# nh13/DWGSIM

Hardware: AMD Instinct MI355X
Metric: M read-pairs/sec (2x150 bp PE) (higher is better)
Workload: dtype u8

## Files before the change

dwgsim_amd/csrc/dw_host.cpp:

```cpp
#include <hip/hip_runtime.h>
#include <math.h>
#include <stdio.h>
#include <stdlib.h>
#include <string.h>
#include <limits.h>
#include <ctype.h>
#include <stdarg.h>
#include <stdint.h>
#include <sys/mman.h>
#include <mutex>
#include <thread>
#include <string>
#include <vector>
#include <algorithm>
#include <array>
#include <stddef.h>
#include <type_traits>
#include "../../include/dwgsim_hip.h"
#include "dw_kernels.hpp"
#include "dw_launch.hpp"
#include "dw_mutin.hpp"
#include "dw_mem.hpp"

using namespace dw;
// ... 1916 lines not shown
    if (c->depth_on && !c->truth_on) { size_t ends = 0; for (int j = 0; j < 2; ++j) if (p.length[j] > 0) ends += n_pairs; P.t_ends = sizeof(TruthEnd) * ends; }
    if (c->truth_on) {
        P.t_qname_max = fixed_max + 120;
        size_t ends = 0, bytes = 0;
        for (int j = 0; j < 2; ++j) if (p.length[j] > 0) { ends += n_pairs; bytes += (size_t)n_pairs * (size_t)(P.t_qname_max + fixed_max + 3 + 10 + 2 + 1 + 10 + 11 + 6 + 11 + 1 + 15 * (size_t)p.length[j]); }
        if (c->truth_md) for (int j = 0; j < 2; ++j) if (p.length[j] > 0) bytes += (size_t)n_pairs * (size_t)(12 + 10 + 2 * (size_t)p.length[j] + 1);
        if (run.truth_bytes) bytes = (size_t)run.truth_bytes;
        else if (c->dbg.truth_cap >= 0 && c->truth_md) bytes = (size_t)std::max<int64_t>(c->dbg.truth_cap, 64);
        P.cap[3] = bytes;
        const bool bfast_src = !L.a.p.has_bwa;
        for (int q = 0; q < (bfast_src ? 1 : f.lpp); ++q) {
            const size_t src_cap = P.cap[bfast_src ? 2 : q];
            P.t_nl[q] = sizeof(uint32_t) * ((src_cap + 4095) / 4096 + 1); P.t_rec[q] = sizeof(uint32_t) * ((bfast_src ? ends : (size_t)n_pairs) + 2);
        }
        P.t_ends = sizeof(TruthEnd) * ends; P.t_len = sizeof(uint32_t) * (ends + 1); P.t_blk = sizeof(uint32_t) * (nblk + 1);
        for (int t = 0; t < N_STREAMS; ++t) if ((uint64_t)P.cap[t] >> 32) P.too_many = true;
    }
    P.block_rand = sizeof(uint32_t) * nblk;
    if (!f.split) P.status = 4 * sizeof(uint64_t) * nblk;
    else { P.split_state = sizeof(uint32_t) * (size_t)f.lds_words * SIM_THREADS * nblk; P.split_hand = 16 * (size_t)SIM_THREADS * nblk; P.split_agg = 16 * nblk; P.split_pre = 32 * nblk; P.split_chunk = 32 * (nblk / 1024 + 1); }
    P.meta = sizeof(uint32_t) * ((size_t)n_pairs + 8);
    P.fail_summ = ((size_t)((n_pairs + 256ull * 64 - 1) / (256ull * 64)) * 4 + 2) * sizeof(uint64_t);
    P.scratch = f.dt == 2 || (f.dt < 2 && f.nthr == SIM_THREADS_LONG);
    if (P.scratch) {
        const int cu_per_xcd = (c->n_cu >= 64 && c->n_cu % 8 == 0) ? c->n_cu / 8 : c->n_cu;
        const bool ion = p.data_type == 2;
        const int per_cu = sim_blocks_per_cu(f.lds, ion ? 8 : 32);
        P.flow_slots = c->dbg.flow_slots > 0 ? c->dbg.flow_slots : cu_per_xcd * per_cu;
        if ((uint64_t)P.flow_slots > (uint64_t)nblk) P.flow_slots = (int32_t)nblk;
        if (ion) {
            const size_t slot_bytes = (size_t)flow_words_per_lane(f.lds_words) * (size_t)SIM_THREADS * sizeof(uint32_t);
            const size_t fit = std::max<size_t>(1, ((size_t)4 << 30) / (slot_bytes * 8));
            if ((size_t)P.flow_slots > fit) P.flow_slots = (int32_t)fit;
        }
        const size_t words = (ion ? (size_t)flow_words_per_lane(f.lds_words) * (size_t)SIM_THREADS : (size_t)f.lds_words * (size_t)SIM_THREADS_LONG) * (size_t)P.flow_slots * 8;
        P.flow_scratch = words * sizeof(uint32_t); P.flow_free = sizeof(uint64_t) * (256 + 8 * nblk);
    }
    P.segs = sizeof(SimSeg) * L.segs.size();
    if (c->gzip_on) {
        size_t chunks = 0;
        for (int t = 0; t < N_STREAMS; ++t) { P.gz_chunks[t] = (size_t)gz_chunks(P.cap[t]); chunks += P.gz_chunks[t]; if (P.cap[t]) P.gz_cap[t] = (size_t)gz_capacity(P.cap[t]); }
        P.gz_status = sizeof(uint64_t) * (chunks ? chunks : 1);
    }
    return P;
}

static int sim_reserve(dwgsim_hip_ctx_t *c, int slot, const SimPlan &P)
{
    Slot &sl = c->slot[slot]; DevMem *out = c->out[slot];
    if (sl.fetch_in_flight) { HIPC(c, hipStreamWaitEvent(c->stream.get(), sl.ev_fetched.get(), 0)); bool grows = false; for (int t = 0; t < N_STREAMS; ++t) if (P.cap[t] + 64 > out[t].cap() && (t < 3 || P.cap[t])) grows = true; if (grows) HIPC(c, hipEventSynchronize(sl.ev_fetched.get())); sl.fetch_in_flight = false; }
    for (int t = 0; t < 3; ++t) if (ensure(c, out[t], P.cap[t] + 64)) return DWGSIM_HIP_ERR_DEVICE;
    if (P.cap[3] && (ensure(c, out[3], P.cap[3] + 64) || ensure(c, c->t_nl[0], P.t_nl[0]) || ensure(c, c->t_nl[1], P.t_nl[1]) || ensure(c, c->t_rec[0], P.t_rec[0]) || ensure(c, c->t_rec[1], P.t_rec[1]) ||
                     ensure(c, c->t_len, P.t_len) || ensure(c, c->t_blk, P.t_blk))) return DWGSIM_HIP_ERR_DEVICE;
    if (ensure(c, c->t_ends, P.t_ends)) return DWGSIM_HIP_ERR_DEVICE;
    if (ensure(c, c->block_rand, P.block_rand) || ensure(c, c->status_all, P.status) ||
        ensure(c, c->split_state, P.split_state) || ensure(c, c->split_hand, P.split_hand) || ensure(c, c->split_agg, P.split_agg) || ensure(c, c->split_pre, P.split_pre) || ensure(c, c->split_chunk, P.split_chunk) ||
        ensure(c, c->meta, P.meta) || ensure(c, c->fail_summ, P.fail_summ) || ensure(c, c->flow_scratch, P.flow_scratch) || ensure(c, c->flow_free, P.flow_free) || ensure(c, sl.segs, P.segs)) return DWGSIM_HIP_ERR_DEVICE;
    HIPC(c, sl.h_segs.reserve(P.segs, P.segs + 64 * sizeof(SimSeg)));
    for (int t = 0; t < N_STREAMS; ++t) if (P.gz_cap[t] && ensure(c, sl.gz_out[t], P.gz_cap[t] + 64)) return DWGSIM_HIP_ERR_DEVICE;
    return ensure(c, sl.gz_status, P.gz_status);
}

static ChainSet sim_chain(dwgsim_hip_ctx_t *c, Slot &sl, const dwgsim_hip_range_t *r, int n, const SimRun &run)
{
    if (run.again) return ChainSet{sl.d_rerun_chain.get<uint64_t>(), 1, 1, 0};
    const dwgsim_hip_range_t *r_first = nullptr, *r_last = nullptr;
    for (int q = 0; q < n; ++q) if (r[q].n_pairs) { if (!r_first) r_first = &r[q]; r_last = &r[q]; }
    if (!r_first) { r_first = &r[0]; r_last = &r[n - 1]; }
    const bool continues = c->chain_contig == r_first->contig && c->chain_next_ii == r_first->first_ii && r_first->first_ii != 0;
    const ChainSet ch{c->d_chain.get<uint64_t>(), run.rand_base != DWGSIM_HIP_RAND_CHAIN ? 1 : 0, (c->has_carry_override || !continues) ? 1 : 0, c->has_carry_override ? c->carry_override : 0};
    c->has_carry_override = false; c->chain_contig = r_last->contig; c->chain_next_ii = r_last->first_ii + r_last->n_pairs;
    if (sl.ranges.data() != r) sl.ranges.assign(r, r + n);
    return ch;
}

static int sim_launch(dwgsim_hip_ctx_t *c, int slot, Launch &L, const SimPlan &P, const ChainSet &ch, const SimRun &run)
{
    Slot &sl = c->slot[slot]; SimArgs &a = L.a; const SimForm &f = L.f; uint64_t *cnt = sl.counters.dev();
    const uint64_t n_pairs = L.n_pairs, rand_base = run.rand_base; const uint32_t nblk = L.nblk;
    for (int t = 0; t < N_STREAMS; ++t) sl.out_bytes[t] = sl.gz_bytes[t] = 0;
    sl.n_pairs = n_pairs; sl.empty = n_pairs == 0; sl.truth_timed = false;
    if (n_pairs == 0) { if (ch.set_rand || ch.set_carry) launch_chain_set(c->stream.get(), ch.words, rand_base, ch.set_rand, ch.carry, ch.set_carry); return DWGSIM_HIP_OK; }
    uint32_t opens = 0; for (const SimSeg &s : L.segs) opens |= s.contig_start;
    memcpy(sl.h_segs.get(), L.segs.data(), P.segs);
    HIPC(c, hipMemcpyAsync(sl.segs.get(), sl.h_segs.get(), P.segs, hipMemcpyHostToDevice, c->stream.get()));
    a.segs = sl.segs.get<SimSeg>(); a.n_seg = (int32_t)L.segs.size(); a.n_blocks = nblk; a.n_pairs = n_pairs; a.chain = ch.words; a.lb_shift = P.lb_shift;
    a.meta = c->meta.get<uint32_t>(); a.block_rand = c->block_rand.get<uint32_t>(); a.counters = cnt;
    for (int t = 0; t < 3; ++t) a.out[t] = c->out[slot][t].get<uint8_t>();
    for (int j = 0; j < 4; ++j) a.status[j] = f.split ? nullptr : c->status_all.get<uint64_t>() + (size_t)j * (size_t)nblk;
    if (f.split) { a.split_state = c->split_state.get<uint32_t>(); a.split_hand = c->split_hand.get<uint32_t>(); a.split_agg = c->split_agg.get<uint32_t>(); a.split_pre = c->split_pre.get<uint64_t>(); a.split_chunk = c->split_chunk.get<uint64_t>(); }
    if (P.scratch) { a.flow_scratch = c->flow_scratch.get<uint32_t>(); a.flow_free = c->flow_free.get<uint64_t>(); a.flow_slots = P.flow_slots; }
    sl.group = c->handles[(size_t)L.g->first_handle].group;
    launch_init(c->stream.get(), cnt, (uint32_t)N_COUNTERS, a.status[0], f.split ? 0 : 4 * (uint64_t)nblk, a.flow_free, a.flow_free ? 256 + 8 * (uint64_t)nblk : 0,
                ch.words, rand_base, ch.set_rand, ch.carry, ch.set_carry);
    HIPC(c, hipEventRecord(sl.ev_k0.get(), c->stream.get()));
    c->dbg.sim_form = (int64_t)f.nthr << 20 | f.lpp << 16 | f.out << 12 | f.dt << 8 | f.wr << 4 | f.split;
    if (!launch_simulate(c->stream.get(), a, f)) { c->err = "simulate: no k_simulate instance for this form"; return DWGSIM_HIP_ERR_FAILED; }
    HIPC(c, hipEventRecord(sl.ev_k1.get(), c->stream.get()));
    sl.cap_mult = c->flow_cap_mult;
    if (!run.again) launch_failrule(c->stream.get(), a.meta, n_pairs, opens, c->fail_summ.get<uint64_t>(), cnt, c->d_chain.get<uint64_t>());
    const bool depth = c->depth_on && !run.again && L.g->depth_valid && !L.g->depth_pos.empty();
    if (P.cap[3] || depth) {
        TruthArgs t; memset(&t, 0, sizeof t);
        sl.truth_timed = true;
        HIPC(c, hipEventRecord(sl.ev_t0.get(), c->stream.get()));
        t.lpp = f.lpp; t.bfast = a.p.has_bwa ? 0 : 1; t.prefix_len = c->read_prefix.empty() ? 0 : (int32_t)c->read_prefix.size() + 1; t.qname_max = P.t_qname_max;
        DepthArgs dp; dp.pos = L.g->mem.d_depth_pos.get<int32_t>(); dp.n = (uint32_t)L.g->depth_pos.size(); dp.cnt = L.g->mem.d_depth_cnt.get<unsigned long long>();
        for (int q = 0; P.cap[3] && q < (t.bfast ? 1 : f.lpp); ++q) {
            const int st = t.bfast ? 2 : q;
            t.src[q] = a.out[st]; t.src_bytes[q] = &cnt[text_len_counter(st)]; t.src_cap[q] = P.cap[st];
            t.nl_count[q] = c->t_nl[q].get<uint32_t>(); t.rec[q] = c->t_rec[q].get<uint32_t>(); t.n_rec[q] = t.bfast ? n_pairs * (uint64_t)f.lpp : n_pairs;
        }
        t.ends = c->t_ends.get<TruthEnd>(); t.line_len = c->t_len.get<uint32_t>(); t.blk = c->t_blk.get<uint32_t>();
        t.out = c->out[slot][3].get<uint8_t>(); t.cap = P.cap[3]; t.total = &cnt[text_len_counter(3)];
        t.md = c->truth_md ? 1 : 0; t.ref = L.g->mem.d_ref.get(); t.fit = &cnt[TRUTH_FIT_COUNTER];
        if (P.cap[3]) launch_truth(c->stream.get(), a, t, depth ? &dp : nullptr);
        else launch_truth_depth(c->stream.get(), a, t, dp);
        HIPC(c, hipEventRecord(sl.ev_t1.get(), c->stream.get()));
    }
    if (c->gzip_on) {
        HIPC(c, hipMemsetAsync(sl.gz_status.get(), 0, P.gz_status, c->stream.get()));
        size_t off = 0;
        for (int t = 0; t < N_STREAMS; ++t) {
            if (P.cap[t] == 0) continue;
            launch_gzip(c->stream.get(), c->out[slot][t].get<uint8_t>(), &cnt[gz_src_len_counter(t, c->truth_md)], P.cap[t], sl.gz_out[t].get<uint8_t>(), P.gz_cap[t], sl.gz_status.get<uint64_t>() + off,
                        &cnt[gz_ticket_counter(t)], &cnt[gz_len_counter(t)], &cnt[STATUS_COUNTER], c->d_crc_table.get<uint32_t>(), c->d_crc_shift.get<uint32_t>());
            off += P.gz_chunks[t];
        }
    }
    HIPC(c, hipEventRecord(sl.ev_end.get(), c->stream.get()));
    HIPC(c, hipGetLastError());
    HIPC(c, hipMemcpyAsync(sl.counters.host(), cnt, N_COUNTERS * sizeof(uint64_t), hipMemcpyDeviceToHost, c->stream.get()));
    HIPC(c, hipEventRecord(sl.ev_done.get(), c->stream.get()));
    sl.pending = true;
    return DWGSIM_HIP_OK;
}

static int sim_enqueue(dwgsim_hip_ctx_t *c, const dwgsim_hip_range_t *r, int n, int slot, const SimRun &run)
{
    if (!c || slot < 0 || slot >= DWGSIM_HIP_SLOTS) { if (c) c->err = "bad simulate arguments"; return DWGSIM_HIP_ERR_ARG; }
    if (c->slot[slot].pending) { c->err = "simulate: the slot still holds a batch that was not waited for"; return DWGSIM_HIP_ERR_STATE; }
    Launch L;
    if (const int rc = sim_resolve(c, r, n, L)) return rc;
    HIPC(c, hipSetDevice(c->device));
    const SimPlan P = sim_plan(c, L, run);
    if (P.too_many) { c->err = "too many pairs in one call"; return DWGSIM_HIP_ERR_ARG; }
    if (L.n_pairs) { if (const int rc = sim_reserve(c, slot, P)) return rc; }
    if (L.n_pairs && c->depth_on && !run.again) { if (const int rc = depth_prepare(c, *L.g)) return rc; }
    return sim_launch(c, slot, L, P, sim_chain(c, c->slot[slot], r, n, run), run);
}

int dwgsim_hip_simulate_ranges_async(dwgsim_hip_ctx_t *c, const dwgsim_hip_range_t *r, int n, uint64_t rand_base, int slot) { return sim_enqueue(c, r, n, slot, SimRun{rand_base, false, 0}); }

int dwgsim_hip_simulate_async(dwgsim_hip_ctx_t *c, int contig, uint64_t first_ii, uint64_t n_pairs, uint64_t rand_base, int slot)
{
    dwgsim_hip_range_t r; memset(&r, 0, sizeof r); r.contig = contig; r.first_ii = first_ii; r.n_pairs = n_pairs;
    return dwgsim_hip_simulate_ranges_async(c, &r, 1, rand_base, slot);
}

static int sim_rerun(dwgsim_hip_ctx_t *c, int slot, uint64_t truth_bytes)
{
    static const int kept[7] = {fail_seg_counter(0), fail_seg_counter(1), fail_seg_counter(2), fail_seg_counter(3), ABORT_COUNTER, CARRY_COUNTER, CHAIN_BASE_COUNTER};
    Slot &sl = c->slot[slot]; uint64_t *h = sl.counters.host();
    uint64_t keep[7]; for (int q = 0; q < 7; ++q) keep[q] = h[kept[q]];
    if (const int rc = sim_enqueue(c, sl.ranges.data(), (int)sl.ranges.size(), slot, SimRun{h[CHAIN_BASE_COUNTER], true, truth_bytes})) return rc;
    HIPC(c, hipEventSynchronize(sl.ev_done.get())); sl.pending = false;
    for (int q = 0; q < 7; ++q) h[kept[q]] = keep[q];
    return DWGSIM_HIP_OK;
}

static int batch_verdict(dwgsim_hip_ctx_t *c, const uint64_t *h)
{
    const uint64_t st = h[STATUS_COUNTER];
    if (st & REGIONS_BIT) { c->err = "dwgsim-hip: no fragment placement satisfied the target regions (-x) after 2^20 tries (the reference would not terminate)\n"; return DWGSIM_HIP_ERR_FAILED; }
    if (st & FLOW_ROOM_BIT) { c->err = "dwgsim-hip: a read outgrew its buffer (or degenerated) in the flow-error model\n"; return DWGSIM_HIP_ERR_FAILED; }
    if ((st & ~(GZIP_ROOM_BIT | TRUTH_ERR_BIT | TRUTH_ROOM_BIT)) || h[ABORT_COUNTER]) return fail_attempts(c);
    if (st & GZIP_ROOM_BIT) { c->err = "dwgsim-hip: the gzip output buffer is too small for this text\n"; return DWGSIM_HIP_ERR_FAILED; }
    if (st & TRUTH_ERR_BIT) { c->err = "dwgsim-hip: the truth SAM could not be made (a read's record or alignment could not be replayed)\n"; return DWGSIM_HIP_ERR_FAILED; }
    if (st & TRUTH_ROOM_BIT) { c->err = "dwgsim-hip: the truth SAM did not fit its buffer\n"; return DWGSIM_HIP_ERR_FAILED; }
    return DWGSIM_HIP_OK;
}

int dwgsim_hip_wait(dwgsim_hip_ctx_t *c, int slot, dwgsim_hip_batch_t *out)
{
    if (!c || slot < 0 || slot >= DWGSIM_HIP_SLOTS) { if (c) c->err = "bad slot"; return DWGSIM_HIP_ERR_ARG; }
    Slot &sl = c->slot[slot];
    if (out) memset(out, 0, sizeof *out);
    if (sl.empty) { sl.pending = false; return DWGSIM_HIP_OK; }
    if (!sl.pending) { c->err = "wait: no batch was enqueued on this slot"; return DWGSIM_HIP_ERR_STATE; }
    HIPC(c, hipSetDevice(c->device));
    HIPC(c, hipEventSynchronize(sl.ev_done.get()));
    sl.pending = false;
    const uint64_t *h = sl.counters.host();
    if ((h[STATUS_COUNTER] & FLOW_ROOM_BIT) && !(h[STATUS_COUNTER] & ~(FLOW_ROOM_BIT | GZIP_ROOM_BIT)) && c->prm.data_type == 2) {
        while (h[STATUS_COUNTER] & FLOW_ROOM_BIT) {
            if (sl.cap_mult >= c->flow_cap_mult) {
                if ((int64_t)flow_base_capacity(c) * (int64_t)c->flow_cap_mult * 2 > (int64_t)FLOW_CAP_MAX) break;
                c->flow_cap_mult *= 2;
            }
            if (const int rc = sim_rerun(c, slot, 0)) return rc;
        }
    }
    if (h[STATUS_COUNTER] == TRUTH_ROOM_BIT && !h[ABORT_COUNTER]) {
        const uint64_t need = h[text_len_counter(3)];
        if (need + 64 >= (1ull << 32)) { c->err = "dwgsim-hip: the truth SAM of one batch would pass 4 GiB with its MD strings (deletions are spelled out): use smaller batches\n"; return DWGSIM_HIP_ERR_UNSUP; }
        if (const int rc = sim_rerun(c, slot, need)) return rc;
        ++c->dbg.truth_reruns;
        if (h[STATUS_COUNTER] & TRUTH_ROOM_BIT) { c->err = "dwgsim-hip: the truth SAM did not fit the room its own scan asked for\n"; return DWGSIM_HIP_ERR_FAILED; }
    }
    if (const int rc = batch_verdict(c, h)) return rc;
    for (int t = 0; t < N_STREAMS; ++t) { sl.out_bytes[t] = h[text_len_counter(t)]; sl.gz_bytes[t] = h[gz_len_counter(t)]; }
    if (!c->truth_on) sl.out_bytes[3] = sl.gz_bytes[3] = 0;
    if (c->dbg.phases) {
        uint64_t tot = 0; for (int k = 0; k < N_PHASES; ++k) tot += h[phase_counter(k)];
        fprintf(stderr, "[phases]");
// ... 332 lines not shown
```

dwgsim_amd/csrc/dw_kernels.hpp:

```cpp
#pragma once
#include <stdint.h>

namespace dw {

constexpr int PAIRS_PER_BLOCK = 128;
constexpr int PLACE_PAIRS = 256;
constexpr int PLACE_LISTS = 64;
#ifndef DW_SIM_THREADS
#define DW_SIM_THREADS 256
#endif
constexpr int SIM_THREADS = DW_SIM_THREADS;
constexpr int FLOW_STACK_WORDS = 4;
constexpr uint32_t FLOW_NEVER = 0xFFFFFFFFu;
constexpr int FLOW_LG_ENTRIES = 257;
constexpr int FLOW_CAP_MAX = 1 << 20;
constexpr int FLOW_STACK_WORDS_MAX = 32;
#ifndef DW_ION_THREADS_SMALL
#define DW_ION_THREADS_SMALL 128
#endif
constexpr int ION_THREADS_SMALL = DW_ION_THREADS_SMALL;
constexpr int SIM_THREADS_LONG = 64;
constexpr int SIM_FIFO_BYTES = 40;
constexpr int SIM_FIFO_BYTES_WIDE = 72;
inline size_t sim_lds_bytes(size_t words_per_lane, size_t lanes, size_t qb_words, bool fifo, size_t fifo_bytes = SIM_FIFO_BYTES) { return ((words_per_lane * lanes + 2 * qb_words + 3) & ~(size_t)3) * 4 + (fifo ? lanes * fifo_bytes : 0); }
// ... 42 lines not shown
    int64_t l;
    SegTab seg;
    const uint32_t *tot4;
    uint32_t cap_bases[2];
};

struct HapRec { uint64_t rec_off; uint32_t hdr_off, hdr_len, base0, n_bases; uint32_t pad_; };
struct ChainEnt { uint32_t pos, info; };
constexpr uint32_t CHAIN_END = 0x80000000u;
constexpr int HAP_WINDOW = 8192;

struct Count { const uint64_t *dev; uint32_t host; };

struct WalkParams {
    double mut_rate, indel_frac, indel_extend;
    uint64_t mut_thr;
    uint64_t gap_r; int32_t gap_s;
    const uint32_t *lg;
    int32_t indel_min, is_hap;
    uint32_t seed;
};

struct SimParams {
    double std_dev, mut_freq, rand_read, quality_std;
    int32_t dist, is_inner, len[2], max_n, strandedness, read_one_strand, amplicons, fixed_quality, data_type;
    int32_t has_bwa, has_bfast;
    uint32_t seed;
    float q_k, q_eps, q_lmin; int32_t q_near1;
};

inline uint64_t flow_ilog2_fixed(uint64_t y, int fb)
{
    const int p = 63 - __builtin_clzll(y);
    uint64_t m = y << (63 - p), frac = 0;
    for (int k = 0; k < fb; ++k) {
        const unsigned __int128 sq = (unsigned __int128)m * m;
        if ((uint64_t)(sq >> 127)) { m = (uint64_t)(sq >> 64); frac = (frac << 1) | 1u; }
        else { m = (uint64_t)(sq >> 63); frac <<= 1; }
    }
    return ((uint64_t)p << fb) | frac;
}
inline void flow_log2_table(uint32_t *lg)
{
    for (int i = 0; i < 256; ++i) lg[i] = (uint32_t)flow_ilog2_fixed(256u + (uint64_t)i, 32);
    lg[256] = 0xFFFFFFFFu;
}
inline void flow_gap_params(uint64_t thr, uint64_t *R, int32_t *s)
{
    *R = 0; *s = 0;
    if (thr == 0 || thr >= 0x100000000ull) return;
    const uint64_t Lq = (32ull << 56) - flow_ilog2_fixed(0x100000000ull - thr, 56);
    const int sh = __builtin_clzll(Lq);
    const unsigned __int128 q = ((unsigned __int128)1 << 127) / (Lq << sh);
    if ((uint64_t)(q >> 64)) { *R = 1ull << 63; *s = 62 - sh; }
    else { *R = (uint64_t)q; *s = 63 - sh; }
}

struct CalibArgs {
    uint32_t seed; int32_t end, len; uint64_t n_reads, first_read, chunk_reads;
    uint64_t thr;
    uint64_t gap_r; int32_t gap_s;
    const uint8_t *flow; int32_t flow_len, lds_words, stack_words;
    uint32_t *scratch;
    uint64_t *counters;
};

constexpr int SUMM_CELLS = 64;
constexpr int SUMM2_CELLS = 1024;

inline constexpr int flow_words_per_lane(int lds_words) { return lds_words | 1; }

struct SimSeg {
    uint32_t first_block;
    uint32_t contig_index;
    int32_t  start, l;
    uint64_t first_ii, n_pairs;
    uint64_t pair_off;
    int64_t  l_place;
    int32_t  reg_off, n_reg;
    uint32_t name_off; int32_t name_fixed_len;
    uint32_t contig_start;
    uint32_t pad_;
};

constexpr int N_COUNTERS = 32;
constexpr int N_STREAMS = 4;
constexpr int N_PHASES = 8;
constexpr int STATUS_COUNTER = 2;
constexpr int TICKET_COUNTER = 0;
constexpr int RETRY_COUNTER = 1;
constexpr int RANDOM_COUNTER = 3;
constexpr int text_len_counter(int t) { return t < 3 ? 4 + t : 7; }
constexpr int phase_counter(int k) { return 8 + k; }
constexpr int fail_seg_counter(int q) { return 16 + q; }
constexpr int ABORT_COUNTER = 20;
constexpr int CARRY_COUNTER = 21;
constexpr int CHAIN_BASE_COUNTER = 22;
constexpr int TRUTH_FIT_COUNTER = 23;
constexpr int gz_len_counter(int t) { return 24 + t; }
constexpr int gz_ticket_counter(int t) { return 28 + t; }
constexpr int gz_src_len_counter(int t, bool truth_md) { return t == 3 && truth_md ? TRUTH_FIT_COUNTER : text_len_counter(t); }
constexpr int PLACE_OPEN_COUNTER = 5;
constexpr int CALIB_ERR_COUNTER = 8;
constexpr int CALIB_LEN_COUNTER = 9;
constexpr int COUNT_BYTE_COUNTER = 15;
constexpr unsigned long long ATTEMPTS_BIT = 1;
constexpr unsigned long long FLOW_ROOM_BIT = 2;
constexpr unsigned long long REGIONS_BIT = 4;
constexpr unsigned long long GZIP_ROOM_BIT = 8;
constexpr unsigned long long PLACE_ROOM_BIT = 16;
constexpr unsigned long long TRUTH_ERR_BIT = 32;
constexpr unsigned long long TRUTH_ROOM_BIT = 64;
constexpr bool counter_claim(uint32_t &seen, int w) { if (w < 0 || w >= N_COUNTERS || (seen >> w & 1u)) return false; seen |= 1u << w; return true; }
constexpr bool slot_counters_ok()
{
    uint32_t seen = 0;
    bool ok = counter_claim(seen, TICKET_COUNTER) && counter_claim(seen, RETRY_COUNTER) && counter_claim(seen, STATUS_COUNTER) && counter_claim(seen, RANDOM_COUNTER) && counter_claim(seen, ABORT_COUNTER) &&
              counter_claim(seen, CARRY_COUNTER) && counter_claim(seen, CHAIN_BASE_COUNTER) && counter_claim(seen, TRUTH_FIT_COUNTER);
    for (int k = 0; k < N_PHASES; ++k) ok = ok && counter_claim(seen, phase_counter(k));
    for (int q = 0; q < 4; ++q) ok = ok && counter_claim(seen, fail_seg_counter(q));
    for (int t = 0; t < N_STREAMS; ++t) ok = ok && counter_claim(seen, text_len_counter(t)) && counter_claim(seen, gz_len_counter(t)) && counter_claim(seen, gz_ticket_counter(t));
    return ok;
}
constexpr bool place_counters_ok() { uint32_t seen = 0; return counter_claim(seen, RETRY_COUNTER) && counter_claim(seen, STATUS_COUNTER) && counter_claim(seen, RANDOM_COUNTER) && counter_claim(seen, PLACE_OPEN_COUNTER); }
constexpr bool context_counters_ok() { uint32_t seen = 0; return counter_claim(seen, STATUS_COUNTER) && counter_claim(seen, CALIB_ERR_COUNTER) && counter_claim(seen, CALIB_LEN_COUNTER) && counter_claim(seen, COUNT_BYTE_COUNTER); }
static_assert(slot_counters_ok(), "slot block: two words collide or one lies behind N_COUNTERS");
static_assert(place_counters_ok(), "place block: two words collide or one lies behind N_COUNTERS");
static_assert(context_counters_ok(), "context block: two words collide or one lies behind N_COUNTERS");

struct SimArgs {
    SimParams p;
    HapDev hap[2];
    const SimSeg *segs; int32_t n_seg; uint32_t n_blocks;
    uint64_t n_pairs;
    const uint64_t *chain;
    const int32_t *reg; int32_t have_regions;
    const uint64_t *e_thr[2];
    const uint16_t *summ[2];
    const uint16_t *summ2[2];
    int32_t place_fast, place_k;
    uint32_t *place_list, *place_list_n; uint32_t place_list_cap;
    uint64_t *range_rand;
    const uint32_t *e_thr32[2];
    int32_t e_full;
    const uint32_t *qbase[2];
    int32_t qb_words;
    const uint8_t *names;
    const uint8_t *rand_fixed; int32_t rand_fixed_len;
    uint32_t *meta;
    uint32_t *block_rand;
    uint64_t *counters;
    uint64_t *status[4];
    uint8_t *out[3];
    int32_t lds_words;
    int32_t cap;
    int32_t ion_lds;
    int32_t flow_stack_words;
    int32_t fifo;
    int32_t sim_threads;
    int32_t flow_len;
    int32_t split;
    uint32_t *split_state;
    uint32_t *split_hand;
    uint32_t *split_agg;
    uint64_t *split_pre;
    uint64_t *split_chunk;
// ... 26 lines not shown
```

dwgsim_amd/csrc/dw_launch.hpp:

```cpp
#pragma once
#include <hip/hip_runtime.h>
#include "dw_kernels.hpp"

namespace dw {
void launch_pack(hipStream_t st, const uint8_t *ascii, uint8_t *ref, uint8_t *h0, uint8_t *h1, int64_t l);
void launch_site_scan_list(hipStream_t st, const uint8_t *refview, int64_t l, SegTab seg, WalkParams wp, uint64_t *status, uint64_t *ticket, int32_t *out, uint32_t cap, uint64_t *n_out);
uint32_t site_scan_blocks(int64_t l);
uint32_t site_scan_block_positions();
void launch_site_scan_slots(hipStream_t st, const uint8_t *refview, int64_t l, SegTab seg, WalkParams wp, int32_t *slots, uint32_t slot_cap, uint32_t *aux, int32_t *out, uint32_t cap, uint64_t *n_out, uint32_t *over);
void launch_mark_dirty(hipStream_t st, const Event *ev, Count n, const int32_t *lo, uint32_t *dirty);
void launch_dirty_chunks(hipStream_t st, bool restore, const uint32_t *dirty, uint32_t n_words, int64_t l_live, const uint8_t *ref, const uint8_t *refview, const uint16_t *refsumm, const uint16_t *refsumm2,
                         uint8_t *cells0, uint8_t *cells1, uint8_t *view0, uint8_t *view1, uint16_t *summ0, uint16_t *summ1, uint16_t *summ2_0, uint16_t *summ2_1);
void launch_scan_excl(hipStream_t st, uint32_t *data, uint32_t n, uint64_t *total_out);
void launch_compact(hipStream_t st, const uint16_t *mask, const uint32_t *block_base, int32_t *out, int64_t l, uint32_t cap);
void launch_events(hipStream_t st, const int32_t *cand, Count n, const uint8_t *ref, SegTab seg, WalkParams wp, Event *ev, uint32_t *max_del);
void walk_debug_seg_min(uint32_t rows);
void launch_resolve(hipStream_t st, Event *ev, Count n, const uint32_t *max_del, uint4 *flags, uint32_t *tot4);
void launch_apply(hipStream_t st, Event *ev, Count n, const uint4 *flags, ContigDev c, WalkParams wp);
void launch_justify_seq(hipStream_t st, const Event *ev, Count n, ContigDev c);
void launch_justify(hipStream_t st, const Event *ev, Count n, ContigDev c, int32_t *lo, int32_t *sufmin, uint8_t *bound);
void launch_mut_debug(hipStream_t st, const uint8_t *ref, const uint8_t *h0, const uint8_t *h1, int64_t l, uint64_t *verdict);
void launch_make_view(hipStream_t st, const uint8_t *cells0, const uint8_t *cells1, int64_t n_cells, int64_t l_live, uint8_t *view0, uint8_t *view1, uint16_t *summ0, uint16_t *summ1, uint16_t *summ2_0, uint16_t *summ2_1);
void launch_apply_patches(hipStream_t st, const int32_t *pos, const uint16_t *cells, uint32_t n, uint8_t *h0, uint8_t *h1);
void launch_collect_mask(hipStream_t st, const uint8_t *h0, const uint8_t *h1, int64_t l, uint16_t *mask, uint32_t *block_count);
void launch_gather(hipStream_t st, const int32_t *pos, uint32_t n, const uint8_t *ref, const uint8_t *h0, const uint8_t *h1, uint32_t *cells);
void launch_hap_len(hipStream_t st, HapDev h, SegTab seg, int64_t l, uint32_t *block_count);
void launch_hap_write(hipStream_t st, HapDev h, SegTab seg, int64_t l, const uint32_t *block_base, const HapRec *rec, uint32_t n_rec, const uint8_t *pool, uint32_t width, uint8_t *text);
void launch_hapchain_count(hipStream_t st, HapDev h, SegTab seg, int64_t l, uint32_t *block_count);
void launch_hapchain_write(hipStream_t st, HapDev h, SegTab seg, int64_t l, const uint32_t *block_base, ChainEnt *out, uint32_t cap);
void launch_place(hipStream_t st, const SimArgs &a);
bool launch_simulate(hipStream_t st, const SimArgs &a, const SimForm &f);
void launch_truth(hipStream_t st, const SimArgs &a, const TruthArgs &t, const DepthArgs *depth);
void launch_truth_depth(hipStream_t st, const SimArgs &a, const TruthArgs &t, const DepthArgs &depth);
int sim_instances(int64_t *out, int cap);
void launch_calibrate(hipStream_t st, const CalibArgs &a);
void launch_failrule(hipStream_t st, const uint32_t *meta, uint64_t n_pairs, uint32_t opens_contig, uint64_t *summ, uint64_t *counters, uint64_t *chain);
void launch_chain_set(hipStream_t st, uint64_t *chain, uint64_t rand_base, int set_rand, uint64_t carry, int set_carry);
void launch_init(hipStream_t st, uint64_t *counters, uint32_t n_counters, uint64_t *z0, uint64_t n0, uint64_t *z1, uint64_t n1, uint64_t *chain, uint64_t rand_base, int set_rand, uint64_t carry, int set_carry);
void launch_selftest_lazy(hipStream_t st, int mode, uint32_t first, uint64_t n, double sigma, float qk, float qeps, float qlmin, int qnear1, uint64_t *out);
uint64_t gz_chunks(uint64_t n);
uint64_t gz_capacity(uint64_t n);
void gz_host_tables(uint32_t *crc_table, uint32_t *crc_shift);
void launch_gzip(hipStream_t st, const uint8_t *text, const uint64_t *n_dev, uint64_t text_cap, uint8_t *out, uint64_t out_cap, uint64_t *status, uint64_t *ticket, uint64_t *total, uint64_t *flags,
                 const uint32_t *crc_table, const uint32_t *crc_shift);
void launch_count_byte(hipStream_t st, const uint8_t *text, uint64_t n, uint32_t byte, uint64_t *out);
void launch_selftest_fp64(hipStream_t st, uint32_t seed, uint64_t n, uint64_t *mism);
void launch_selftest_text(hipStream_t st, uint64_t first, uint64_t n, uint64_t stride, uint64_t *out);
void launch_selftest_gap(hipStream_t st, const uint32_t *lg, uint64_t R, int sR, uint32_t first, uint64_t n, uint32_t g_lo, uint32_t g_cnt, uint32_t *chg, uint64_t *out);
}
```

dwgsim_amd/csrc/dw_simulate.hip:

```cpp
#include <algorithm>
#include "dw_read.hpp"
#include "dw_launch.hpp"

#ifndef DW_PART
#define DW_PART -1
#endif
#define DW_HAS(part) (DW_PART == -1 || DW_PART == (part))
#if DW_HAS(0)
#include "dw_truth.hpp"
#endif
#ifndef DW_SIM_WAVES
#define DW_SIM_WAVES 5
#endif
#ifndef DW_SOLID_WAVES
#define DW_SOLID_WAVES 4
#endif
#ifndef DW_SIM_WAVES_BOTH
#define DW_SIM_WAVES_BOTH 4
#endif
#ifndef DW_SIMB_WAVES
#define DW_SIMB_WAVES 6
#endif
#ifndef DW_IONA_WAVES
#define DW_IONA_WAVES 4
// ... 992 lines not shown
}
__global__ void __launch_bounds__(64) k_split_scan2(SimArgs a, int lpp)
{
    const uint32_t nch = (a.n_blocks + 1023u) / 1024u;
    uint64_t run[3] = {0, 0, 0};
    for (uint32_t base = 0; base < nch; base += 64u) {
        const uint32_t c = base + threadIdx.x;
        uint64_t v[3] = {0, 0, 0};
        if (c < nch) for (int k = 0; k < 3; ++k) v[k] = a.split_chunk[4 * (size_t)c + k];
        uint64_t inc[3];
#pragma unroll
        for (int k = 0; k < 3; ++k) {
            uint64_t x = v[k];
#pragma unroll
            for (int d = 1; d < 64; d <<= 1) { const uint32_t ol = (uint32_t)__shfl_up((int)(uint32_t)x, d), oh = (uint32_t)__shfl_up((int)(uint32_t)(x >> 32), d); if (lane_id() >= d) x += ((uint64_t)oh << 32) | ol; }
            inc[k] = x;
        }
        if (c < nch) for (int k = 0; k < 3; ++k) a.split_chunk[4 * (size_t)c + k] = run[k] + inc[k] - v[k];
        for (int k = 0; k < 3; ++k) { const uint32_t lo = (uint32_t)__shfl((int)(uint32_t)inc[k], 63), hi = (uint32_t)__shfl((int)(uint32_t)(inc[k] >> 32), 63); run[k] += ((uint64_t)hi << 32) | lo; }
    }
    if (threadIdx.x == 0) {
        const uint64_t H = hex_digits_sum(a.chain[0], run[0]), G1 = run[1] + H, G2 = run[2] + (lpp == 2 ? H : 0ull);
        const uint64_t nreads = a.n_pairs * (uint64_t)((a.p.len[1] > 0) ? 2 : 1);
        a.counters[RANDOM_COUNTER] = run[0];
        a.counters[text_len_counter(0)] = a.p.has_bwa ? G1 : 0;
        a.counters[text_len_counter(1)] = a.p.has_bwa ? G2 : 0;
        a.counters[text_len_counter(2)] = !a.p.has_bfast ? 0 : G1 + G2 - 2 * nreads;
    }
}

struct FailSeg { uint64_t P, S; uint32_t R, bad; };
DW_DEV FailSeg failseg_join(const FailSeg &a, const FailSeg &b)
{
    FailSeg r;
    r.bad = a.bad | b.bad | ((a.R && a.S + b.P > (uint64_t)MAX_ATTEMPTS) ? 1u : 0u);
    r.P = a.R ? a.P : a.P + b.P;
    r.S = b.R ? b.S : a.S + b.S;
    r.R = a.R | b.R;
    return r;
}
DW_DEV FailSeg failseg_wave_join(FailSeg x, int cnt)
{
    const int lane = lane_id();
#pragma unroll
    for (int d = 1; d < 64; d <<= 1) {
        FailSeg o;
        o.P = ((uint64_t)(uint32_t)__shfl_down((int)(uint32_t)(x.P >> 32), d) << 32) | (uint32_t)__shfl_down((int)(uint32_t)x.P, d);
        o.S = ((uint64_t)(uint32_t)__shfl_down((int)(uint32_t)(x.S >> 32), d) << 32) | (uint32_t)__shfl_down((int)(uint32_t)x.S, d);
        o.R = (uint32_t)__shfl_down((int)x.R, d); o.bad = (uint32_t)__shfl_down((int)x.bad, d);
        if ((lane & (2 * d - 1)) == 0 && lane + d < cnt) x = failseg_join(x, o);
    }
    return x;
}
constexpr int FAIL_PAIRS_PER_THREAD = 64;
__global__ void __launch_bounds__(256) k_failrule_a(const uint32_t *__restrict__ meta, uint64_t n_pairs, const uint64_t *__restrict__ counters, uint64_t *__restrict__ summ)
{
    __shared__ FailSeg seg[4];
    if (counters[RETRY_COUNTER] == 0) return;
    const uint64_t first = ((uint64_t)blockIdx.x * 256 + threadIdx.x) * FAIL_PAIRS_PER_THREAD;
    FailSeg s{0, 0, 0, 0};
    for (int q4 = 0; q4 < FAIL_PAIRS_PER_THREAD && first + q4 < n_pairs; q4 += 4) {
        const uint4 v = *reinterpret_cast<const uint4 *>(meta + first + q4);
        const uint32_t mm[4] = {v.x, v.y, v.z, v.w};
#pragma unroll
        for (int u = 0; u < 4; ++u) {
            if (first + q4 + u >= n_pairs) break;
            const uint32_t m = mm[u];
            if (m & 0x40000000u) s = failseg_join(s, FailSeg{0, 0, 1, 0});
            FailSeg one{m & 0x3fffffffu, 0, (m >> 31) ? 0u : 1u, 0};
            if (!one.R) one.S = one.P;
            s = failseg_join(s, one);
        }
    }
    s = failseg_wave_join(s, 64);
    if ((threadIdx.x & 63) == 0) seg[threadIdx.x >> 6] = s;
    __syncthreads();
    if (threadIdx.x == 0) {
        FailSeg t = seg[0];
        for (int k = 1; k < 4; ++k) t = failseg_join(t, seg[k]);
        summ[4 * (uint64_t)blockIdx.x + 0] = t.P; summ[4 * (uint64_t)blockIdx.x + 1] = t.S;
        summ[4 * (uint64_t)blockIdx.x + 2] = t.R; summ[4 * (uint64_t)blockIdx.x + 3] = t.bad;
    }
}
__global__ void __launch_bounds__(64) k_failrule_b(const uint64_t *__restrict__ summ, uint32_t n_blocks, uint64_t n_pairs, uint32_t opens_contig, uint64_t *__restrict__ counters, uint64_t *__restrict__ chain)
{
    FailSeg t{0, 0, (counters[RANDOM_COUNTER] < n_pairs || opens_contig) ? 1u : 0u, 0};
    if (counters[RETRY_COUNTER] != 0) {
        const uint32_t per = (n_blocks + 63) / 64, b0 = threadIdx.x * per, b1 = b0 + per < n_blocks ? b0 + per : n_blocks;
        FailSeg x{0, 0, 0, 0};
        for (uint32_t b = b0; b < b1; ++b) {
            const FailSeg nx{summ[4 * (uint64_t)b], summ[4 * (uint64_t)b + 1], (uint32_t)summ[4 * (uint64_t)b + 2], (uint32_t)summ[4 * (uint64_t)b + 3]};
            x = (b == b0) ? nx : failseg_join(x, nx);
        }
        t = failseg_wave_join(x, per ? (int)((n_blocks + per - 1) / per) : 0);
    }
    if (threadIdx.x == 0) {
        const uint64_t carry = chain[1];
        const FailSeg all = failseg_join(FailSeg{carry, carry, 0, 0}, t);
        counters[fail_seg_counter(0)] = t.P; counters[fail_seg_counter(1)] = t.S; counters[fail_seg_counter(2)] = t.R; counters[fail_seg_counter(3)] = t.bad;
        counters[ABORT_COUNTER] = (all.bad || all.P > (uint64_t)MAX_ATTEMPTS || all.S > (uint64_t)MAX_ATTEMPTS) ? 1 : 0;
        counters[CARRY_COUNTER] = all.S;
        chain[1] = all.S;
        counters[CHAIN_BASE_COUNTER] = chain[0];
        chain[0] += counters[RANDOM_COUNTER];
    }
}
void launch_failrule(hipStream_t st, const uint32_t *meta, uint64_t n_pairs, uint32_t opens_contig, uint64_t *summ, uint64_t *counters, uint64_t *chain)
{
    const uint32_t nb = cdiv(n_pairs, 256ull * FAIL_PAIRS_PER_THREAD);
    hipLaunchKernelGGL(k_failrule_a, dim3(nb), dim3(256), 0, st, meta, n_pairs, counters, summ);
    hipLaunchKernelGGL(k_failrule_b, dim3(1), dim3(64), 0, st, summ, nb, n_pairs, opens_contig, counters, chain);
}
__global__ void __launch_bounds__(64) k_chain_set(uint64_t *chain, uint64_t rand_base, int set_rand, uint64_t carry, int set_carry)
{
    if (threadIdx.x != 0) return;
    if (set_rand) chain[0] = rand_base;
    if (set_carry) chain[1] = carry;
}
void launch_chain_set(hipStream_t st, uint64_t *chain, uint64_t rand_base, int set_rand, uint64_t carry, int set_carry)
{
    hipLaunchKernelGGL(k_chain_set, dim3(1), dim3(64), 0, st, chain, rand_base, set_rand, carry, set_carry);
}
__global__ void __launch_bounds__(256) k_launch_init(uint64_t *counters, uint32_t n_counters, uint64_t *z0, uint64_t n0, uint64_t *z1, uint64_t n1, uint64_t *chain, uint64_t rand_base, int set_rand, uint64_t carry, int set_carry)
{
    const uint64_t i = (uint64_t)blockIdx.x * 256 + threadIdx.x, stride = (uint64_t)gridDim.x * 256;
    if (i < n_counters) counters[i] = 0;
    for (uint64_t k = i; k < n0; k += stride) z0[k] = 0;
    for (uint64_t k = i; k < n1; k += stride) z1[k] = 0;
    if (i == 0) { if (set_rand) chain[0] = rand_base; if (set_carry) chain[1] = carry; }
}
void launch_init(hipStream_t st, uint64_t *counters, uint32_t n_counters, uint64_t *z0, uint64_t n0, uint64_t *z1, uint64_t n1, uint64_t *chain, uint64_t rand_base, int set_rand, uint64_t carry, int set_carry)
{
    const uint64_t most = n0 > n1 ? n0 : n1, want = (most + 255) / 256;
    hipLaunchKernelGGL(k_launch_init, dim3((uint32_t)(want < 1 ? 1 : want > 2048 ? 2048 : want)), dim3(256), 0, st, counters, n_counters, z0, n0, z1, n1, chain, rand_base, set_rand, carry, set_carry);
}
__global__ void __launch_bounds__(256) k_count_byte(const uint8_t *__restrict__ text, uint64_t n, uint32_t byte, uint64_t *out)
{
    const uint32_t pat = byte * 0x01010101u;
    uint32_t cnt = 0;
    const uint64_t nvec = n / 16;
    for (uint64_t v = (uint64_t)blockIdx.x * 256 + threadIdx.x; v < nvec; v += (uint64_t)gridDim.x * 256) {
        const uint4 q = reinterpret_cast<const uint4 *>(text)[v];
        const uint32_t w[4] = {q.x ^ pat, q.y ^ pat, q.z ^ pat, q.w ^ pat};
#pragma unroll
        for (int k = 0; k < 4; ++k) cnt += (uint32_t)__popc(~(((w[k] & 0x7F7F7F7Fu) + 0x7F7F7F7Fu) | w[k] | 0x7F7F7F7Fu));
    }
    if (blockIdx.x == 0 && threadIdx.x == 0) for (uint64_t q = nvec * 16; q < n; ++q) cnt += text[q] == byte;
    const uint32_t s = wave_sum_u32(cnt);
    if ((threadIdx.x & 63) == 0 && s) atomicAdd((unsigned long long *)out, (unsigned long long)s);
}
void launch_count_byte(hipStream_t st, const uint8_t *text, uint64_t n, uint32_t byte, uint64_t *out)
{
    hipLaunchKernelGGL(k_count_byte, dim3(4096), dim3(256), 0, st, text, n, byte, out);
}
void launch_place(hipStream_t st, const SimArgs &a)
{
    hipLaunchKernelGGL(k_place, dim3(a.n_blocks), dim3(PLACE_PAIRS), 0, st, a);
    const uint32_t per_list = (uint32_t)std::min<uint64_t>(16, std::max<uint64_t>(1, ((uint64_t)a.place_list_cap + 1023) / 1024));
    hipLaunchKernelGGL(k_place_rest, dim3(PLACE_LISTS * per_list), dim3(128), 0, st, a);
    launch_scan_excl(st, a.block_rand, a.n_blocks, &a.counters[RANDOM_COUNTER]);
    hipLaunchKernelGGL(k_range_counts, dim3(cdiv((uint64_t)a.n_seg, 256)), dim3(256), 0, st, a);
}
void launch_split_scan(hipStream_t st, const SimArgs &a, int lpp)
{
    hipLaunchKernelGGL(k_split_scan1, dim3(cdiv(a.n_blocks, 1024)), dim3(1024), 0, st, a);
    hipLaunchKernelGGL(k_split_scan2, dim3(1), dim3(64), 0, st, a, lpp);
}
#endif

#if DW_HAS(4)
__global__ void __launch_bounds__(PAIRS_PER_BLOCK) k_calibrate(CalibArgs a)
{
    DW_DYN_SHARED(uint32_t, dyn_lds);
    __shared__ FlowTables s_ft;
    const int tid = (int)threadIdx.x, nthr = PAIRS_PER_BLOCK;
    if (tid < 64) s_ft.flow[tid] = a.flow[tid];
    __syncthreads();
    fill_flow_tables(s_ft, a.flow_len, tid, nthr, a.flow);
    __syncthreads();
    const uint64_t jj = a.first_read + (uint64_t)blockIdx.x * PAIRS_PER_BLOCK + (uint64_t)tid;
    uint32_t *buf = a.scratch + (size_t)blockIdx.x * ((size_t)a.lds_words * nthr) + tid;
    const int capb = 16 * a.lds_words;
    int32_t n_err = 0; int s_out = 0;
    const bool live = jj < a.n_reads;
    const RngKey key{a.seed, 0u};
    const uint32_t dom = D_CALIB + (uint32_t)a.end;
    if (live) {
        const int h0 = ((capb - a.len) & ~7) >> 3;
        for (int w = 0; w * 8 < a.len; ++w) {
            const U4 q0 = rng_block(key, dom, jj, 0, 0, (uint32_t)(2 * w)), q1 = rng_block(key, dom, jj, 0, 0, (uint32_t)(2 * w + 1));
            const uint32_t rw[8] = {q0.x, q0.y, q0.z, q0.w, q1.x, q1.y, q1.z, q1.w};
            uint32_t pairs = 0;
#pragma unroll
            for (int b = 0; b < 8; ++b) if (w * 8 + b < a.len) pairs |= (rw[b] >> 30) << (2 * b);
            const int h = h0 + w;
            reinterpret_cast<uint16_t *>(buf + (h >> 1) * nthr)[h & 1] = (uint16_t)pairs;
        }
    }
    {
        FlowRng rg; rg.seed = a.seed; rg.contig = 0; rg.dom = dom; rg.att = 1; rg.evt = 0; rg.s = 0; rg.ii = jj; rg.w0 = rg.w1 = rg.w2 = rg.w3 = 0;
        const int so = flow_errors(live, rg, s_ft, a.flow_len, a.thr, a.gap_r, a.gap_s, buf, dyn_lds + tid, nthr, 2 * a.stack_words, a.len, 0, capb, &n_err);
        if (live) { s_out = so; if (s_out < 0) { atomicOr((unsigned long long *)&a.counters[STATUS_COUNTER], FLOW_ROOM_BIT); s_out = 0; n_err = 0; } }
    }
    const uint32_t es = wave_sum_u32((uint32_t)n_err), ls = wave_sum_u32((uint32_t)s_out);
    if ((tid & 63) == 0) { atomicAdd((unsigned long long *)&a.counters[CALIB_ERR_COUNTER], (unsigned long long)es); atomicAdd((unsigned long long *)&a.counters[CALIB_LEN_COUNTER], (unsigned long long)ls); }
}
void launch_calibrate(hipStream_t st, const CalibArgs &a)
{
    hipLaunchKernelGGL(k_calibrate, dim3(cdiv(std::min(a.chunk_reads, a.n_reads - a.first_read), (uint64_t)PAIRS_PER_BLOCK)), dim3(PAIRS_PER_BLOCK), (size_t)a.stack_words * PAIRS_PER_BLOCK * 4, st, a);
}
#endif

#define DW_SIM_OUTS(X, LPP, DT, NTHR, WR, SPLIT) X(LPP, 1, DT, NTHR, WR, SPLIT) X(LPP, 2, DT, NTHR, WR, SPLIT) X(LPP, 3, DT, NTHR, WR, SPLIT)
#define DW_SIM_PART_1(X)  DW_SIM_OUTS(X, 2, 0, 256, 0, 0) DW_SIM_OUTS(X, 2, 0, 256, 1, 0)
#define DW_SIM_PART_2(X)  DW_SIM_OUTS(X, 1, 0, 256, 0, 0) DW_SIM_OUTS(X, 1, 0, 256, 1, 0)
#define DW_SIM_PART_3(X)  DW_SIM_OUTS(X, 2, 2, 256, 1, 0)
#define DW_SIM_PART_4(X)  DW_SIM_OUTS(X, 1, 2, 256, 1, 0)
// ... 67 lines not shown
```

Before: 1504.

## Pass small segment tables as kernel args and mirror counters from failrule epilogue

When a batch has at most four segments, the segment table is now packed into the init kernel's arguments and written to device memory there, instead of going through a host staging memcpy and an H2D copy. When no truth, depth or gzip stage follows, the final failrule kernel writes all counters straight into the pinned host buffer with system-scope stores, so the separate D2H counter copy is dropped. Together these remove two small DMA operations per batch. The cost is a larger kernarg block and a reliance on coherent system-scope stores to host memory being visible once the completion event fires.

```diff
diff --git a/dwgsim_amd/csrc/dw_host.cpp b/dwgsim_amd/csrc/dw_host.cpp
--- a/dwgsim_amd/csrc/dw_host.cpp
+++ b/dwgsim_amd/csrc/dw_host.cpp
@@ -2022,8 +2022,11 @@
     sl.n_pairs = n_pairs; sl.empty = n_pairs == 0; sl.truth_timed = false;
     if (n_pairs == 0) { if (ch.set_rand || ch.set_carry) launch_chain_set(c->stream.get(), ch.words, rand_base, ch.set_rand, ch.carry, ch.set_carry); return DWGSIM_HIP_OK; }
     uint32_t opens = 0; for (const SimSeg &s : L.segs) opens |= s.contig_start;
-    memcpy(sl.h_segs.get(), L.segs.data(), P.segs);
-    HIPC(c, hipMemcpyAsync(sl.segs.get(), sl.h_segs.get(), P.segs, hipMemcpyHostToDevice, c->stream.get()));
+    const bool segs_inline = L.segs.size() <= (size_t)SimSegInline::MAX;
+    if (!segs_inline) {
+        memcpy(sl.h_segs.get(), L.segs.data(), P.segs);
+        HIPC(c, hipMemcpyAsync(sl.segs.get(), sl.h_segs.get(), P.segs, hipMemcpyHostToDevice, c->stream.get()));
+    }
     a.segs = sl.segs.get<SimSeg>(); a.n_seg = (int32_t)L.segs.size(); a.n_blocks = nblk; a.n_pairs = n_pairs; a.chain = ch.words; a.lb_shift = P.lb_shift;
     a.meta = c->meta.get<uint32_t>(); a.block_rand = c->block_rand.get<uint32_t>(); a.counters = cnt;
     for (int t = 0; t < 3; ++t) a.out[t] = c->out[slot][t].get<uint8_t>();
@@ -2032,14 +2035,15 @@
     if (P.scratch) { a.flow_scratch = c->flow_scratch.get<uint32_t>(); a.flow_free = c->flow_free.get<uint64_t>(); a.flow_slots = P.flow_slots; }
     sl.group = c->handles[(size_t)L.g->first_handle].group;
     launch_init(c->stream.get(), cnt, (uint32_t)N_COUNTERS, a.status[0], f.split ? 0 : 4 * (uint64_t)nblk, a.flow_free, a.flow_free ? 256 + 8 * (uint64_t)nblk : 0,
-                ch.words, rand_base, ch.set_rand, ch.carry, ch.set_carry);
+                ch.words, rand_base, ch.set_rand, ch.carry, ch.set_carry, L.segs.data(), segs_inline ? (uint32_t)L.segs.size() : 0u, sl.segs.get<SimSeg>());
     HIPC(c, hipEventRecord(sl.ev_k0.get(), c->stream.get()));
     c->dbg.sim_form = (int64_t)f.nthr << 20 | f.lpp << 16 | f.out << 12 | f.dt << 8 | f.wr << 4 | f.split;
     if (!launch_simulate(c->stream.get(), a, f)) { c->err = "simulate: no k_simulate instance for this form"; return DWGSIM_HIP_ERR_FAILED; }
     HIPC(c, hipEventRecord(sl.ev_k1.get(), c->stream.get()));
     sl.cap_mult = c->flow_cap_mult;
-    if (!run.again) launch_failrule(c->stream.get(), a.meta, n_pairs, opens, c->fail_summ.get<uint64_t>(), cnt, c->d_chain.get<uint64_t>());
     const bool depth = c->depth_on && !run.again && L.g->depth_valid && !L.g->depth_pos.empty();
+    const bool mirror_by_epilogue = !run.again && !(P.cap[3] || depth) && !c->gzip_on;
+    if (!run.again) launch_failrule(c->stream.get(), a.meta, n_pairs, opens, c->fail_summ.get<uint64_t>(), cnt, c->d_chain.get<uint64_t>(), mirror_by_epilogue ? sl.counters.host() : nullptr);
     if (P.cap[3] || depth) {
         TruthArgs t; memset(&t, 0, sizeof t);
         sl.truth_timed = true;
@@ -2070,7 +2074,7 @@
     }
     HIPC(c, hipEventRecord(sl.ev_end.get(), c->stream.get()));
     HIPC(c, hipGetLastError());
-    HIPC(c, hipMemcpyAsync(sl.counters.host(), cnt, N_COUNTERS * sizeof(uint64_t), hipMemcpyDeviceToHost, c->stream.get()));
+    if (!mirror_by_epilogue) HIPC(c, hipMemcpyAsync(sl.counters.host(), cnt, N_COUNTERS * sizeof(uint64_t), hipMemcpyDeviceToHost, c->stream.get()));
     HIPC(c, hipEventRecord(sl.ev_done.get(), c->stream.get()));
     sl.pending = true;
     return DWGSIM_HIP_OK;
diff --git a/dwgsim_amd/csrc/dw_kernels.hpp b/dwgsim_amd/csrc/dw_kernels.hpp
--- a/dwgsim_amd/csrc/dw_kernels.hpp
+++ b/dwgsim_amd/csrc/dw_kernels.hpp
@@ -148,6 +148,8 @@
     uint32_t contig_start;
     uint32_t pad_;
 };
+struct SimSegInline { static constexpr int MAX = 4, WORDS = MAX * (int)(sizeof(SimSeg) / sizeof(uint64_t)); uint64_t w[WORDS]; };
+static_assert(sizeof(SimSeg) % sizeof(uint64_t) == 0 && sizeof(SimSegInline) + 128 <= 4096, "whole words, and an argument block far inside the kernarg limit");
 
 constexpr int N_COUNTERS = 32;
 constexpr int N_STREAMS = 4;
diff --git a/dwgsim_amd/csrc/dw_launch.hpp b/dwgsim_amd/csrc/dw_launch.hpp
--- a/dwgsim_amd/csrc/dw_launch.hpp
+++ b/dwgsim_amd/csrc/dw_launch.hpp
@@ -34,9 +34,10 @@
 void launch_truth_depth(hipStream_t st, const SimArgs &a, const TruthArgs &t, const DepthArgs &depth);
 int sim_instances(int64_t *out, int cap);
 void launch_calibrate(hipStream_t st, const CalibArgs &a);
-void launch_failrule(hipStream_t st, const uint32_t *meta, uint64_t n_pairs, uint32_t opens_contig, uint64_t *summ, uint64_t *counters, uint64_t *chain);
+void launch_failrule(hipStream_t st, const uint32_t *meta, uint64_t n_pairs, uint32_t opens_contig, uint64_t *summ, uint64_t *counters, uint64_t *chain, uint64_t *mirror);
 void launch_chain_set(hipStream_t st, uint64_t *chain, uint64_t rand_base, int set_rand, uint64_t carry, int set_carry);
-void launch_init(hipStream_t st, uint64_t *counters, uint32_t n_counters, uint64_t *z0, uint64_t n0, uint64_t *z1, uint64_t n1, uint64_t *chain, uint64_t rand_base, int set_rand, uint64_t carry, int set_carry);
+void launch_init(hipStream_t st, uint64_t *counters, uint32_t n_counters, uint64_t *z0, uint64_t n0, uint64_t *z1, uint64_t n1, uint64_t *chain, uint64_t rand_base, int set_rand, uint64_t carry, int set_carry,
+                 const SimSeg *segs, uint32_t n_seg, SimSeg *seg_dst);
 void launch_selftest_lazy(hipStream_t st, int mode, uint32_t first, uint64_t n, double sigma, float qk, float qeps, float qlmin, int qnear1, uint64_t *out);
 uint64_t gz_chunks(uint64_t n);
 uint64_t gz_capacity(uint64_t n);
diff --git a/dwgsim_amd/csrc/dw_simulate.hip b/dwgsim_amd/csrc/dw_simulate.hip
--- a/dwgsim_amd/csrc/dw_simulate.hip
+++ b/dwgsim_amd/csrc/dw_simulate.hip
@@ -1098,7 +1098,8 @@
         summ[4 * (uint64_t)blockIdx.x + 2] = t.R; summ[4 * (uint64_t)blockIdx.x + 3] = t.bad;
     }
 }
-__global__ void __launch_bounds__(64) k_failrule_b(const uint64_t *__restrict__ summ, uint32_t n_blocks, uint64_t n_pairs, uint32_t opens_contig, uint64_t *__restrict__ counters, uint64_t *__restrict__ chain)
+DW_DEV void mirror_store(uint64_t *p, uint64_t v) { __hip_atomic_store(p, v, __ATOMIC_RELAXED, __HIP_MEMORY_SCOPE_SYSTEM); }
+__global__ void __launch_bounds__(64) k_failrule_b(const uint64_t *__restrict__ summ, uint32_t n_blocks, uint64_t n_pairs, uint32_t opens_contig, uint64_t *counters, uint64_t *__restrict__ chain, uint64_t *mirror)
 {
     FailSeg t{0, 0, (counters[RANDOM_COUNTER] < n_pairs || opens_contig) ? 1u : 0u, 0};
     if (counters[RETRY_COUNTER] != 0) {
@@ -1114,18 +1115,26 @@
         const uint64_t carry = chain[1];
         const FailSeg all = failseg_join(FailSeg{carry, carry, 0, 0}, t);
         counters[fail_seg_counter(0)] = t.P; counters[fail_seg_counter(1)] = t.S; counters[fail_seg_counter(2)] = t.R; counters[fail_seg_counter(3)] = t.bad;
-        counters[ABORT_COUNTER] = (all.bad || all.P > (uint64_t)MAX_ATTEMPTS || all.S > (uint64_t)MAX_ATTEMPTS) ? 1 : 0;
+        const uint64_t counters_abort = (all.bad || all.P > (uint64_t)MAX_ATTEMPTS || all.S > (uint64_t)MAX_ATTEMPTS) ? 1 : 0;
+        counters[ABORT_COUNTER] = counters_abort;
         counters[CARRY_COUNTER] = all.S;
         chain[1] = all.S;
-        counters[CHAIN_BASE_COUNTER] = chain[0];
+        const uint64_t chain_base = chain[0];
+        counters[CHAIN_BASE_COUNTER] = chain_base;
         chain[0] += counters[RANDOM_COUNTER];
-    }
-}
-void launch_failrule(hipStream_t st, const uint32_t *meta, uint64_t n_pairs, uint32_t opens_contig, uint64_t *summ, uint64_t *counters, uint64_t *chain)
+        if (mirror) {
+            mirror_store(&mirror[fail_seg_counter(0)], t.P); mirror_store(&mirror[fail_seg_counter(1)], t.S); mirror_store(&mirror[fail_seg_counter(2)], t.R); mirror_store(&mirror[fail_seg_counter(3)], t.bad);
+            mirror_store(&mirror[ABORT_COUNTER], counters_abort); mirror_store(&mirror[CARRY_COUNTER], all.S); mirror_store(&mirror[CHAIN_BASE_COUNTER], chain_base);
+        }
+    }
+    static_assert(fail_seg_counter(0) == 16 && fail_seg_counter(3) == 19 && ABORT_COUNTER == 20 && CARRY_COUNTER == 21 && CHAIN_BASE_COUNTER == 22, "the words k_failrule_b writes: 16 .. 22");
+    if (mirror && threadIdx.x < (uint32_t)N_COUNTERS && (threadIdx.x < 16u || threadIdx.x > 22u)) mirror_store(&mirror[threadIdx.x], counters[threadIdx.x]);
+}
+void launch_failrule(hipStream_t st, const uint32_t *meta, uint64_t n_pairs, uint32_t opens_contig, uint64_t *summ, uint64_t *counters, uint64_t *chain, uint64_t *mirror)
 {
     const uint32_t nb = cdiv(n_pairs, 256ull * FAIL_PAIRS_PER_THREAD);
     hipLaunchKernelGGL(k_failrule_a, dim3(nb), dim3(256), 0, st, meta, n_pairs, counters, summ);
-    hipLaunchKernelGGL(k_failrule_b, dim3(1), dim3(64), 0, st, summ, nb, n_pairs, opens_contig, counters, chain);
+    hipLaunchKernelGGL(k_failrule_b, dim3(1), dim3(64), 0, st, summ, nb, n_pairs, opens_contig, counters, chain, mirror);
 }
 __global__ void __launch_bounds__(64) k_chain_set(uint64_t *chain, uint64_t rand_base, int set_rand, uint64_t carry, int set_carry)
 {
@@ -1137,18 +1146,30 @@
 {
     hipLaunchKernelGGL(k_chain_set, dim3(1), dim3(64), 0, st, chain, rand_base, set_rand, carry, set_carry);
 }
-__global__ void __launch_bounds__(256) k_launch_init(uint64_t *counters, uint32_t n_counters, uint64_t *z0, uint64_t n0, uint64_t *z1, uint64_t n1, uint64_t *chain, uint64_t rand_base, int set_rand, uint64_t carry, int set_carry)
+__global__ void __launch_bounds__(256) k_launch_init(uint64_t *counters, uint32_t n_counters, uint64_t *z0, uint64_t n0, uint64_t *z1, uint64_t n1, uint64_t *chain, uint64_t rand_base, int set_rand, uint64_t carry, int set_carry,
+                                                     SimSegInline segs, uint64_t *seg_dst, uint32_t seg_words)
 {
     const uint64_t i = (uint64_t)blockIdx.x * 256 + threadIdx.x, stride = (uint64_t)gridDim.x * 256;
     if (i < n_counters) counters[i] = 0;
+    if (i < seg_words) {
+#pragma unroll
+        for (int q = 0; q < SimSegInline::WORDS; ++q) if (i == (uint64_t)q) seg_dst[q] = segs.w[q];
+    }
     for (uint64_t k = i; k < n0; k += stride) z0[k] = 0;
     for (uint64_t k = i; k < n1; k += stride) z1[k] = 0;
     if (i == 0) { if (set_rand) chain[0] = rand_base; if (set_carry) chain[1] = carry; }
 }
-void launch_init(hipStream_t st, uint64_t *counters, uint32_t n_counters, uint64_t *z0, uint64_t n0, uint64_t *z1, uint64_t n1, uint64_t *chain, uint64_t rand_base, int set_rand, uint64_t carry, int set_carry)
-{
+void launch_init(hipStream_t st, uint64_t *counters, uint32_t n_counters, uint64_t *z0, uint64_t n0, uint64_t *z1, uint64_t n1, uint64_t *chain, uint64_t rand_base, int set_rand, uint64_t carry, int set_carry,
+                 const SimSeg *segs, uint32_t n_seg, SimSeg *seg_dst)
+{
+    SimSegInline si{};
+    if (n_seg > (uint32_t)SimSegInline::MAX) n_seg = 0;
+    const uint32_t seg_words = n_seg * (uint32_t)(sizeof(SimSeg) / sizeof(uint64_t));
+    const uint64_t *src = reinterpret_cast<const uint64_t *>(segs);
+    for (uint32_t q = 0; q < seg_words; ++q) si.w[q] = src[q];
     const uint64_t most = n0 > n1 ? n0 : n1, want = (most + 255) / 256;
-    hipLaunchKernelGGL(k_launch_init, dim3((uint32_t)(want < 1 ? 1 : want > 2048 ? 2048 : want)), dim3(256), 0, st, counters, n_counters, z0, n0, z1, n1, chain, rand_base, set_rand, carry, set_carry);
+    hipLaunchKernelGGL(k_launch_init, dim3((uint32_t)(want < 1 ? 1 : want > 2048 ? 2048 : want)), dim3(256), 0, st, counters, n_counters, z0, n0, z1, n1, chain, rand_base, set_rand, carry, set_carry,
+                       si, reinterpret_cast<uint64_t *>(seg_dst), seg_words);
 }
 __global__ void __launch_bounds__(256) k_count_byte(const uint8_t *__restrict__ text, uint64_t n, uint32_t byte, uint64_t *out)
 {
```

Result: no change. 1515 (median of 3 runs) (+0.7%).
